# NVIDIA/tensorrt-laboratory

Measured on NVIDIA H100. Metric: ResNet-50 fp16 b=8 inferences/sec, higher is better.
Workload: dtype f16

## Files before the change

### tensorrt_laboratory_b200/csrc/engine.cu

```cuda
#include <cuda.h>
#include <cuda_runtime.h>
#include <stdarg.h>
#include <stdio.h>
#include <stdlib.h>
#include <string.h>

#include <algorithm>
#include <map>
#include <memory>
#include <mutex>
#include <string>
#include <vector>

#include "../../include/b200infer.h"
#include "kernels.h"
#include "plan_format.h"

#include "b2_internal.h"

namespace b2i {
thread_local std::string g_err;
int fail(int code, const char* fmt, ...) {
    char buf[1024];
    va_list ap;
// ... 42 lines not shown
        if (cudaGetDriverEntryPoint("cuTensorMapEncodeIm2col", &fn, cudaEnableDefault, &q) != cudaSuccess || !fn) {
            g_driver_status = 2;
            return;
        }
        g_encode_im2col = reinterpret_cast<EncodeIm2colFn>(fn);
        cudaDriverGetVersion(&g_driver_version);
    });
    return g_driver_status;
}

size_t align_up(size_t v, size_t a) { return (v + a - 1) / a * a; }
constexpr size_t kSplitWorkspaceBytes = 12u << 20;
constexpr int kMaxSplitTiles = 4096;

int env_int(const char* name, int dflt) {
    const char* v = getenv(name);
    return v ? atoi(v) : dflt;
}

struct Tensor {
    std::string name;
    uint32_t kind, h, w, c, c_phys;
    int binding;
    float scale = 0.f;
    size_t item_bytes = 0;
    size_t offset = 0;
    int def = -1, last_use = -1;
};

struct Op {
    b2plan::OpRec r;
    std::string name;
    int side_join = -1;
    int kh() const { return int(r.k); }
    int kw() const { return int(r.kw ? r.kw : r.k); }
    int sh() const { return int(r.stride); }
    int sw() const { return int(r.kw ? r.stride_w : r.stride); }
    int ph() const { return int(r.pad_); }
    int pw_lo() const { return int(r.kw ? r.pad_w_lo : r.pad_); }
    int pw_hi() const { return int(r.kw ? r.pad_w_hi : r.pad_); }
    double algo_k() const { return r.ceil_mode ? double(r.ceil_mode) : double(r.cin) * r.taps; }
};

struct Binding {
    std::string name;
    bool is_input;
    int dtype;
    int tensor;
    int nd;
    int32_t dims[8];
    size_t item_bytes;
};

enum LKind { L_INPUT_CAST, L_CONV_TC, L_CONV_SIMT, L_MAXPOOL, L_AVGPOOL, L_FC, L_SOFTMAX, L_OUTPUT_CAST, L_NET, L_TAIL, L_QUANTIZE, L_CONV_I8, L_AVGPOOL_I8, L_OUTPUT_CAST_I8 };

struct NetRun {
    b2k::NetArgs args{};
    int ctas = 0;
    int first_op = 0, last_op = 0;
    void* d_blob = nullptr;
    ~NetRun() {
        if (d_blob) cudaFree(d_blob);
    }
};

struct Launch {
    LKind kind;
    std::string name;
    double flops = 0, bytes = 0;
    b2k::ConvLaunch conv;
    b2k::SimtConvArgs simt;
    const void* in = nullptr;
    void* out = nullptr;
    const void* w = nullptr;
    const float* bias = nullptr;
    int in_binding = -1, out_binding = -1;
    bool src_half = false;
    int max_blocks = 0;
    int side_join = -1;
    std::shared_ptr<NetRun> net;
    b2k::TailArgs tail{};
    b2k::I8ConvLaunch i8{};
    float qscale = 0.f;
    int C_in_phys = 0;
    bool net_member = false;
    int N = 0, C = 0, H = 0, W = 0, C_phys = 0, Ho = 0, Wo = 0, k = 0, stride = 0, pad = 0, K = 0, Cout = 0;
};

struct Segment {
    int begin = 0, end = 0;
    bool graphable = false;
    cudaGraphExec_t exec = nullptr;
};
struct BindPatch {
    int launch = -1;
    cudaGraphNode_t node = nullptr;
    cudaKernelNodeParams np{};
    std::vector<void*> params;
    int n_params = 0;
    int in_index = -1, out_index = -1;
    void* in_value = nullptr;
    void* out_value = nullptr;
    b2k::TailArgs tail{};
    bool is_tail = false;
};
struct Plan {
    int batch = 0;
    bool has_net = false;
    std::vector<Launch> launches;
    std::vector<Segment> segments;
    bool graph_failed = false;
    cudaGraph_t graph = nullptr;
    cudaGraphExec_t exec = nullptr;
    std::vector<BindPatch> patches;
    ~Plan() {
        for (Segment& sg : segments)
            if (sg.exec) cudaGraphExecDestroy(sg.exec);
        if (exec) cudaGraphExecDestroy(exec);
        if (graph) cudaGraphDestroy(graph);
    }
};

}

struct ConvConfig {
    int bn, stages, splits;
    double est_us;
    int sps = 1;
    int ws = 0;
    int cn = 1;
    int halo = 0;
};
static bool stage_depth_useful(int bn, int kb, int st, int kpc) {
    const int stgs[4] = {1, 2, 4, 8};
    int cover = 0, deepest = 0;
// ... 14 lines not shown
    void* user = nullptr;
};

struct b2_engine {
    b2_runtime* rt = nullptr;
    b2_alloc_fn alloc = nullptr;
    b2_free_fn free_ = nullptr;
    void* alloc_user = nullptr;
    std::string name;
    int precision = 0, max_batch = 0;
    std::vector<Tensor> tensors;
    std::vector<Op> ops;
    std::vector<Binding> bindings;
    uint8_t* d_payload = nullptr;
    size_t payload_bytes = 0;
    size_t arena_bytes = 0;
    size_t act_bytes = 0;
    int device = -1;
    bool inspect_only = false;
    double flops_per_item = 0;
    std::mutex tune_mutex;
    std::mutex tune_run_mutex;
    std::map<std::pair<int, int>, ConvConfig> tuned;
    bool tune_cache_loaded = false;
    std::map<int, float> requant_r;
    bool tactics_from_plan = false;
    bool tuned_at_load = false;
    bool half() const { return precision != B2_PREC_FP32; }
    bool int8() const { return precision == B2_PREC_INT8; }
};

struct b2_context {
    b2_engine* e = nullptr;
    uint8_t* scratch = nullptr;
    struct ScratchState {
        std::map<int, std::unique_ptr<Plan>> plans;
    };
    std::map<uint8_t*, ScratchState> states;
    ScratchState* cur = nullptr;
    int* d_counters = nullptr;
    int use_graph = 1;
    int force_simt = 0;
    int force_im2col = 0;
    int force_bn = 0;
    int force_stages = 0;
    int force_splits = 0;
    int force_sps = 0;
    int force_halo = 0;
    int force_cn = 0;
    int force_ws = 0;
    int pdl_trigger = 1;
    int no_pack = 0;
    int no_fold = 0;
    int autotune = 4;
    int fork = 0;
    int net = 0;
    int net_ctas = 0;
    int net_bn = 0;
    int net_stages = 0;
    int i8_bn = 0;
    int i8_stages = 0;
    int fuse_tail = 1;
    int input_ctas = 0;
    int* d_tail_ctrl = nullptr;
    cudaStream_t side = nullptr;
    cudaEvent_t fork_ev = nullptr, join_ev = nullptr;
};

namespace {

std::string fixed_str(const char* p, size_t n) {
    size_t len = 0;
    while (len < n && p[len]) ++len;
    return std::string(p, len);
}

int parse_blob(const void* blob, size_t nbytes, b2_engine* e, const uint8_t** payload) {
    using namespace b2plan;
    if (!blob || nbytes < sizeof(Header)) return fail(B2_EINVAL, "plan: blob too small (%zu bytes)", nbytes);
    const uint8_t* base = static_cast<const uint8_t*>(blob);
    Header h;
    memcpy(&h, base, sizeof h);
    if (memcmp(h.magic, kMagic, 8) != 0) return fail(B2_EINVAL, "plan: bad magic (not a B2ENGINE blob)");
    if (h.version != kVersion) return fail(B2_EINVAL, "plan: version %u, this library reads %u", h.version, kVersion);
    if (h.precision > 2) return fail(B2_EINVAL, "plan: unknown precision %u", h.precision);
    if (h.max_batch == 0 || h.max_batch > 4096) return fail(B2_EINVAL, "plan: bad max_batch %u", h.max_batch);
    const size_t tbl = sizeof(Header) + size_t(h.n_tensors) * sizeof(TensorRec) + size_t(h.n_ops) * sizeof(OpRec) +
                       size_t(h.n_bindings) * sizeof(BindingRec);
    if (tbl > nbytes || h.payload_offset < tbl || h.payload_offset > nbytes || h.payload_bytes > nbytes - h.payload_offset)
        return fail(B2_EINVAL, "plan: truncated (tables %zu, payload %llu+%llu, blob %zu)", tbl,
                    (unsigned long long)h.payload_offset, (unsigned long long)h.payload_bytes, nbytes);
    e->name = fixed_str(h.name, 64);
    e->precision = h.precision;
    e->max_batch = h.max_batch;
    e->payload_bytes = h.payload_bytes;
    const size_t elt = h.precision == B2_PREC_FP32 ? 4 : 2;
    const uint8_t* p = base + sizeof(Header);
    for (uint32_t i = 0; i < h.n_tensors; ++i, p += sizeof(TensorRec)) {
        TensorRec r;
        memcpy(&r, p, sizeof r);
        Tensor t;
        t.name = fixed_str(r.name, 64);
        t.kind = r.kind;
        t.h = r.h, t.w = r.w, t.c = r.c, t.c_phys = r.c_phys;
        t.binding = r.binding;
        t.scale = h.precision == B2_PREC_INT8 ? r.scale : 0.f;
// ... 228 lines not shown
    if (g_driver_version <= 13010 && img_bytes * uint64_t(N) < 131072)
        reinterpret_cast<uint64_t*>(map)[1] &= ~(1ull << 21);
    return B2_OK;
}

static int g_sms = 132;

ConvConfig pick_conv_config(int M, int cout_phys, int kblocks, int kb, bool residual, const b2_context* c, bool honor_forced) {
    const int m_tiles = (M + 127) / 128;
    ConvConfig best{0, 0, 1, 1e30};
    const int bns[4] = {256, 128, 64, 32};
    const int stgs[4] = {1, 2, 4, 8};
    for (int bn : bns) {
        if (cout_phys % bn) continue;
        if (honor_forced && c->force_bn && bn != c->force_bn) continue;
        const int tiles = m_tiles * (cout_phys / bn);
        for (int splits = 1; splits <= 8; ++splits) {
            if (c->force_splits ? splits != c->force_splits : splits != 1) continue;
            if (splits > 1 && (kb != 64 || kblocks / splits < 4 || tiles * splits > 160 || tiles > kMaxSplitTiles ||
                               size_t(tiles) * splits * 128 * bn * 4 > kSplitWorkspaceBytes))
                continue;
            const int kpc = (kblocks + splits - 1) / splits;
            if (splits > 1 && (splits - 1) * kpc >= kblocks) continue;
            for (int st : stgs) {
                if (!b2k::conv_config_exists(bn, kb, st)) continue;
                if (b2k::conv_smem_bytes(bn, st, residual) > 227 * 1024) continue;
                if (honor_forced && c->force_stages && st != c->force_stages) continue;
                if (!(honor_forced && c->force_stages) && !stage_depth_useful(bn, kb, st, kpc)) continue;
                const double smem = b2k::conv_smem_bytes(bn, st, residual);
                int per_sm = int(227.0 * 1024 / smem);
                per_sm = std::min(per_sm, bn <= 64 ? 2 : 1);
                per_sm = std::max(1, std::min(per_sm, 8));
                const int ctas = tiles * splits;
                const int waves = (ctas + g_sms * per_sm - 1) / (g_sms * per_sm);
                const int sharing = std::max(1, std::min(per_sm, (ctas + g_sms - 1) / g_sms));
                const double stage_bytes = 16384.0 + bn * 128.0;
                const double t_kb = std::max(stage_bytes / (70000.0 / sharing), 1.0 / st);
                double t_epi = 0.6 + bn / 64.0 * 0.4 + (residual ? 0.4 : 0.0);
                if (splits > 1) t_epi += 1.0 + 0.3 * splits;
                const double t_cta = 2.0 + kpc * t_kb + t_epi;
                double total = waves * t_cta;
                const double traffic = double(ctas) * kpc * stage_bytes;
                total = std::max(total, traffic / 5.0e6 + 2.0);
                if (total < best.est_us) best = ConvConfig{bn, st, splits, total};
            }
        }
    }
    return best;
}

bool conv_is_row_folded(const b2_context* c, const Op& op) {
    const b2plan::OpRec& r = op.r;
    return !c->no_fold && r.cin_phys == 8 && op.kw() * 8 * 2 == 64 && op.sw() == 1 && op.pw_lo() == 0 && op.pw_hi() == 0;
}
int conv_kb(const b2_context* c, const Op& op) {
    if (op.r.cin_phys % 64 == 0) return 64;
    return conv_is_row_folded(c, op) ? 32 : 8;
}
int conv_num_kblocks(const b2_context* c, const Op& op) {
    const b2plan::OpRec& r = op.r;
    if (r.cin_phys % 64 == 0) return int(r.taps) * (int(r.cin_phys) / 64);
    if (conv_is_row_folded(c, op)) return (op.kh() + 1) / 2;
    return (int(r.taps_phys) + 7) / 8;
}

int conv_halo_rows(const b2_context* c, const Op& op) {
    const b2plan::OpRec& r = op.r;
    const Tensor& ti = c->e->tensors[r.in];
    const Tensor& to = c->e->tensors[r.out];
    if (r.cin_phys % 64 || r.cout_phys % 64 || op.kh() != 3 || op.kw() != 3 || op.sh() != 1 || op.sw() != 1 || op.ph() != 1 ||
        op.pw_lo() != 1 || op.pw_hi() != 1 || r.res >= 0 || !(r.relu & 2) || c->no_pack || ti.h != to.h || ti.w != to.w)
        return 0;
    const int wp = int(to.w) + 2;
    if (wp > 128) return 0;
    return std::min(128 / wp, int(to.h));
}

int make_conv_launch(b2_context* c, const Op& op, int batch, const ConvConfig& cfg, b2k::ConvLaunch* out) {
    b2_engine* e = c->e;
    const b2plan::OpRec& r = op.r;
    const Tensor& ti = e->tensors[r.in];
    const Tensor& to = e->tensors[r.out];
    auto tptr = [&](int idx) -> uint8_t* { return c->scratch + e->tensors[idx].offset; };
    const uint8_t* w = e->d_payload + r.w_off;
    const int M = batch * int(to.h) * int(to.w);
    const bool kb64 = r.cin_phys % 64 == 0;
    const bool fold = conv_is_row_folded(c, op);
    b2k::ConvLaunch& cl = *out;
    memset(&cl, 0, sizeof cl);
    cl.kb = conv_kb(c, op);
    cl.grid_m = (M + 127) / 128;
    const int nkb = conv_num_kblocks(c, op);
    cl.bn = cfg.bn;
    cl.stages = cfg.stages;
    cl.sps = cfg.sps > 0 ? cfg.sps : 1;
    cl.grid_n = int(r.cout_phys) / cl.bn;
    cl.ws_ctas = cfg.ws;
    cl.cn = (cfg.cn > 1 && cfg.ws == 0 && cl.kb == 64 && cl.grid_n % cfg.cn == 0 &&
             b2k::conv_cluster_config_exists(cl.bn, cl.stages, cl.sps, cfg.cn)) ? cfg.cn : 1;
    cl.args.cn = cl.cn;
    cl.args.tiles_m = cl.grid_m;
    cl.args.tiles_n = cl.grid_n;
    b2k::ConvArgs& a = cl.args;
    a.splits = cfg.splits;
    a.kb_per_split = (nkb + cfg.splits - 1) / cfg.splits;
    a.workspace = reinterpret_cast<float*>(c->scratch + e->act_bytes);
// ... 646 lines not shown
                L.bytes = double(batch) * t.h * t.w * (t.c * 4.0 + t.c_phys * elt);
                break;
            }
            case b2plan::OP_QUANTIZE: {
                const Tensor& ti = e->tensors[r.in];
                const Tensor& to = e->tensors[r.out];
                L.kind = L_QUANTIZE;
                L.in = tptr(r.in), L.out = tptr(r.out);
                L.C = ti.c, L.H = ti.h, L.W = ti.w, L.C_in_phys = ti.c_phys, L.C_phys = to.c_phys;
                L.qscale = float(1.0 / double(to.scale));
                L.bytes = double(batch) * (ti.item_bytes + to.item_bytes);
                break;
            }
            case b2plan::OP_OUTPUT_CAST: {
                const Tensor& t = e->tensors[r.in];
                L.kind = t.scale > 0.f ? L_OUTPUT_CAST_I8 : L_OUTPUT_CAST;
                L.qscale = t.scale;
                L.in = tptr(r.in);
                L.out_binding = r.binding;
                L.C = t.c, L.H = t.h, L.W = t.w, L.C_phys = t.c_phys;
                L.bytes = double(batch) * t.h * t.w * (t.c * 4.0 + t.c_phys * elt);
                break;
            }
            case b2plan::OP_CONV: {
                const Tensor& ti = e->tensors[r.in];
                const Tensor& to = e->tensors[r.out];
                const uint8_t* w = e->d_payload + r.w_off;
                const float* bias = reinterpret_cast<const float*>(e->d_payload + r.b_off);
                const int M = batch * int(to.h) * int(to.w);
                L.flops = 2.0 * M * r.cout * op.algo_k();
                L.bytes = double(batch) * (ti.item_bytes + to.item_bytes * (r.res >= 0 ? 2 : 1)) + double(r.w_bytes);
                const bool kb64 = r.cin_phys % 64 == 0;
                const bool kb8 = r.cin_phys == 8;
                const bool tc_ok = half && !c->force_simt && (kb64 || kb8) && r.cout_phys % 32 == 0 &&
                                   (kb64 || r.taps_phys % 2 == 0);
                if (r.relu & 4) {
                    L.kind = L_CONV_I8;
                    const int m_tiles = (batch * int(e->tensors[r.out].h * e->tensors[r.out].w) + 127) / 128;
                    int bn = 128, st = m_tiles * (int(r.cout_phys) / 128) >= 2 * g_sms ? 1 : 2;
                    if (c->autotune) {
                        std::lock_guard<std::mutex> lock(e->tune_mutex);
                        tune_cache_load(e);
                        const int op_index = int(&op - &e->ops[0]);
                        auto it = e->tuned.find({op_index, batch});
                        if (it == e->tuned.end()) it = e->tuned.find({op_index, e->max_batch});
                        if (it != e->tuned.end()) bn = it->second.bn, st = it->second.stages;
                    }
                    if (c->i8_bn > 0) bn = c->i8_bn;
                    if (c->i8_stages > 0) st = c->i8_stages;
                    if (int(r.cout_phys) % bn) bn = 128;
                    if (!b2k::conv_i8_config_exists(bn, st)) bn = 128, st = 2;
                    int rc = make_i8_conv_launch(c, op, batch, bn, st, &L.i8);
                    if (rc) return rc;
                } else if (tc_ok) {
                    L.kind = L_CONV_TC;
                    const int kbsz = conv_kb(c, op);
                    const int nkb = conv_num_kblocks(c, op);
                    ConvConfig cfg = pick_conv_config(M, int(r.cout_phys), nkb, kbsz, r.res >= 0, c, true);
                    if (cfg.bn == 0)
                        cfg = pick_conv_config(M, int(r.cout_phys), nkb, kbsz, r.res >= 0, c, false);
                    if (cfg.bn == 0) return fail(B2_EINVAL, "conv %s: no kernel configuration", op.name.c_str());
                    if (c->force_sps == 2 && b2k::conv_config_exists(cfg.bn, kbsz, cfg.stages, 2) &&
                        b2k::conv_smem_bytes(cfg.bn, cfg.stages, r.res >= 0, 2) <= 227 * 1024)
                        cfg.sps = 2;
                    if (c->force_ws > 0 && kbsz == 64 && (r.relu & 2) && cfg.splits == 1 &&
                        b2k::conv_ws_config_exists(cfg.bn, cfg.stages, cfg.sps) &&
                        b2k::conv_ws_smem(cfg.bn, cfg.stages, cfg.sps, r.res >= 0) <= 227 * 1024)
                        cfg.ws = std::min(((M + 127) / 128) * (int(r.cout_phys) / cfg.bn), c->force_ws > 1 ? c->force_ws : g_sms);
                    if (c->force_halo > 0 && conv_halo_rows(c, op) && b2k::conv_halo_config_exists(cfg.bn) && cfg.splits == 1 &&
                        int(r.cin_phys) / 64 <= 8 && b2k::conv_halo_smem(cfg.bn, int(to.w), conv_halo_rows(c, op), int(r.cin_phys) / 64) <= 227 * 1024)
                        cfg.halo = 1, cfg.ws = 0, cfg.cn = 1;
                    if (c->force_cn > 1 && kbsz == 64 && cfg.ws == 0 && !cfg.halo && (int(r.cout_phys) / cfg.bn) % c->force_cn == 0) cfg.cn = c->force_cn;
                    const bool forced = c->force_bn || c->force_stages || c->force_splits || c->force_sps;
                    const int op_index = int(&op - &e->ops[0]);
                    const bool net_ok = c->net && !forced && kbsz == 64 && (r.relu & 2) && !c->no_pack && r.cout_phys % 64 == 0 &&
                                        c->force_ws <= 0 && c->force_cn <= 0 && c->force_halo <= 0 && !c->force_im2col;
                    if (net_ok) {
                        int bn = (r.cout_phys % 128 == 0) ? 128 : 64;
                        if (c->net_bn == 64) bn = 64;
                        cfg = ConvConfig{bn, 4, 1, 0.0, 1, 0, 1};
                        cfg.halo = 0;
                        L.net_member = true;
                    } else if (!forced && c->autotune) {
                        std::lock_guard<std::mutex> lock(e->tune_mutex);
                        tune_cache_load(e);
                        auto it = e->tuned.find({op_index, batch});
                        if (it == e->tuned.end()) it = e->tuned.find({op_index, e->max_batch});
                        if (it != e->tuned.end() && tactic_applies(c, op, batch, it->second)) cfg = it->second;
                    }
                    if (op.side_join >= 0 && cfg.splits > 1) cfg.splits = 1;
                    int rc = make_conv_launch(c, op, batch, cfg, &L.conv);
                    if (rc) return rc;
                } else {
                    L.kind = L_CONV_SIMT;
                    b2k::SimtConvArgs& a = L.simt;
                    memset(&a, 0, sizeof a);
                    a.in = tptr(r.in), a.w = w, a.bias = bias;
                    a.residual = r.res >= 0 ? tptr(r.res) : nullptr;
                    a.out = tptr(r.out);
                    a.N = batch, a.H = int(ti.h), a.W = int(ti.w), a.Cin = int(r.cin), a.Cin_phys = int(r.cin_phys);
                    a.Ho = int(to.h), a.Wo = int(to.w), a.Cout = int(r.cout), a.Cout_phys = int(r.cout_phys);
                    a.kh = op.kh(), a.kw = op.kw(), a.taps_phys = int(r.taps_phys);
                    a.stride_h = op.sh(), a.stride_w = op.sw(), a.pad_h = op.ph(), a.pad_w = op.pw_lo();
                    a.relu = int(r.relu & 1);
                    a.w_packed = int((r.relu >> 1) & 1);
                }
// ... 38 lines not shown
            }
            case b2plan::OP_SOFTMAX: {
                const Tensor& ti = e->tensors[r.in];
                const Tensor& to = e->tensors[r.out];
                L.kind = L_SOFTMAX;
                L.in = tptr(r.in);
                L.in_binding = ti.binding;
                L.out = tptr(r.out);
                L.out_binding = to.binding;
                L.C = int(ti.c);
                L.bytes = double(batch) * ti.c * 8.0;
                break;
            }
            default:
                return fail(B2_EINVAL, "op %s: unknown type", op.name.c_str());
        }
        plan->launches.push_back(std::move(L));
    }
    int rc = fuse_net_runs(c, plan.get(), batch);
    if (rc) return rc;
    fuse_tail(c, plan.get(), batch);
    {
        const std::vector<Launch>& ls = plan->launches;
        size_t i = 0;
        while (i < ls.size()) {
            const bool dep = ls[i].in_binding >= 0 || ls[i].out_binding >= 0;
            size_t j = i + 1;
            if (!dep)
                while (j < ls.size() && ls[j].in_binding < 0 && ls[j].out_binding < 0) ++j;
            Segment sg;
            sg.begin = int(i), sg.end = int(j);
            sg.graphable = !dep && (j - i) >= 3 && !plan->has_net;
            plan->segments.push_back(sg);
            i = j;
        }
    }
    *out = plan.get();
    c->cur->plans[batch] = std::move(plan);
    return B2_OK;
}

int run_launch(const b2_engine* e, const Launch& L, void* const* bindings, cudaStream_t s) {
    const bool half = e->half();
    const void* in = L.in_binding >= 0 ? bindings[L.in_binding] : L.in;
    void* out = L.out_binding >= 0 ? bindings[L.out_binding] : L.out;
    switch (L.kind) {
        case L_INPUT_CAST:
            if (L.k == 2) return b2k::launch_input_cast_s2d(in, L.src_half, out, L.N, L.C, L.H, L.W, L.pad, L.stride, L.max_blocks, s);
            return b2k::launch_input_cast(in, L.src_half, out, L.N, L.C, L.H, L.W, L.C_phys, half, L.max_blocks, s);
        case L_OUTPUT_CAST:
            return b2k::launch_output_cast(in, static_cast<float*>(out), L.N, L.C, L.H, L.W, L.C_phys, half, s);
        case L_CONV_TC:
            return b2k::launch_conv_f16_tcgen05(L.conv, s);
        case L_CONV_SIMT:
            return b2k::launch_conv_simt(L.simt, half, s);
        case L_MAXPOOL:
            return b2k::launch_maxpool(in, out, L.N, L.H, L.W, L.C_phys, L.Ho, L.Wo, L.k, L.stride, L.pad, half, s);
        case L_AVGPOOL:
            return b2k::launch_avgpool(in, out, L.N, L.H * L.W, L.C_phys, half, s);
        case L_FC:
            return b2k::launch_fc(in, L.w, L.bias, static_cast<float*>(out), L.N, L.K, L.Cout, half, s);
        case L_SOFTMAX:
            return b2k::launch_softmax(static_cast<const float*>(in), static_cast<float*>(out), L.N, L.C, s);
        case L_NET:
            return b2k::launch_net_f16_tcgen05(L.net->args, L.net->ctas, s);
        case L_QUANTIZE:
            return b2k::launch_quantize_h_to_i8(in, out, static_cast<long long>(L.N) * L.H * L.W, L.C, L.C_in_phys, L.C_phys, L.qscale, s);
        case L_CONV_I8:
            return b2k::launch_conv_i8_tcgen05(L.i8, s);
        case L_AVGPOOL_I8:
            return b2k::launch_avgpool_i8(in, out, L.N, L.H * L.W, L.C, L.C_in_phys, L.C_phys, L.qscale, s);
        case L_OUTPUT_CAST_I8:
            return b2k::launch_output_cast_i8(in, static_cast<float*>(out), L.N, L.C, L.H, L.W, L.C_phys, L.qscale, s);
        case L_TAIL: {
            b2k::TailArgs t = L.tail;
            t.out = static_cast<float*>(out);
            return b2k::launch_tail_f16(t, s);
        }
    }
    return int(cudaErrorInvalidValue);
}

int run_range(b2_context* c, const Plan& plan, size_t first, size_t last, void* const* bindings, cudaStream_t s);
int run_all(b2_context* c, const Plan& plan, void* const* bindings, cudaStream_t s) {
    return run_range(c, plan, 0, plan.launches.size(), bindings, s);
}
int run_range(b2_context* c, const Plan& plan, size_t first, size_t last, void* const* bindings, cudaStream_t s) {
    const b2_engine* e = c->e;
    bool fork = c->fork != 0;
    if (fork && !c->side) {
        if (cudaStreamCreateWithFlags(&c->side, cudaStreamNonBlocking) != cudaSuccess ||
            cudaEventCreateWithFlags(&c->fork_ev, cudaEventDisableTiming) != cudaSuccess ||
            cudaEventCreateWithFlags(&c->join_ev, cudaEventDisableTiming) != cudaSuccess) {
            cudaGetLastError();
            fork = false;
        }
    }
    int pending_join = -1;
    for (size_t i = first; i < last; ++i) {
        const Launch& L = plan.launches[i];
        if (pending_join == int(i)) {
            B2_CUDA(cudaStreamWaitEvent(s, c->join_ev, 0));
            pending_join = -1;
        }
        int rc;
        if (fork && pending_join < 0 && L.side_join > int(i) && L.side_join < int(last)) {
// ... 323 lines not shown
    c->cur = c->scratch ? &c->states[c->scratch] : nullptr;
}

void b2_context_destroy(b2_context* c) {
    if (!c) return;
    drop_cached(c);
    if (c->d_counters) cudaFree(c->d_counters);
    if (c->side) cudaStreamDestroy(c->side);
    if (c->fork_ev) cudaEventDestroy(c->fork_ev);
    if (c->join_ev) cudaEventDestroy(c->join_ev);
    delete c;
}

int b2_context_set_device_memory(b2_context* c, void* scratch) {
    if (!c || !scratch) return fail(B2_EINVAL, "null context or scratch");
    if (reinterpret_cast<uintptr_t>(scratch) % 256 != 0) return fail(B2_EINVAL, "scratch must be 256-byte aligned (cudaMalloc alignment)");
    if (c->states.size() >= 32 && c->states.find(static_cast<uint8_t*>(scratch)) == c->states.end()) drop_cached(c);
    c->scratch = static_cast<uint8_t*>(scratch);
    c->cur = &c->states[c->scratch];
    return B2_OK;
}

int b2_context_set_option(b2_context* c, const char* key, int value) {
    if (!c || !key) return fail(B2_EINVAL, "null context or key");
    const std::string k(key);
    if (k == "graph") {
        c->use_graph = value;
        return B2_OK;
    }
    if (k == "pdl") {
        b2k::set_pdl(value != 0);
        value = 0;
    } else if (k == "simt") c->force_simt = value;
    else if (k == "im2col") c->force_im2col = value;
    else if (k == "bn") c->force_bn = value;
    else if (k == "stages") c->force_stages = value;
    else if (k == "splits") c->force_splits = value;
    else if (k == "sps") c->force_sps = value;
    else if (k == "ws") c->force_ws = value;
    else if (k == "cn") c->force_cn = value;
    else if (k == "halo") c->force_halo = value;
    else if (k == "fork") c->fork = value;
    else if (k == "net") c->net = value;
    else if (k == "net_ctas") c->net_ctas = value;
    else if (k == "net_bn") c->net_bn = value;
    else if (k == "net_stages") c->net_stages = value;
    else if (k == "fuse_tail") c->fuse_tail = value;
    else if (k == "i8_bn") c->i8_bn = value;
    else if (k == "i8_stages") c->i8_stages = value;
    else if (k == "input_ctas") c->input_ctas = value;
    else if (k == "pdl_trigger") c->pdl_trigger = value;
    else if (k == "autotune") c->autotune = value;
    else if (k == "no_fold") c->no_fold = value;
    else return fail(B2_EINVAL, "unknown option '%s'", key);
    drop_cached(c);
    return B2_OK;
}

int b2_context_nb_launches(b2_context* c, int batch) {
    if (!c) return -1;
    Plan* plan = nullptr;
    if (build_plan(c, batch, &plan)) return -1;
    return int(plan->launches.size());
}

int b2_engine_tune(b2_engine* e, int streams, int all_batches) {
    if (!e) return fail(B2_EINVAL, "null engine");
    if (e->inspect_only) return fail(B2_ESTATE, "engine was loaded with b2_engine_inspect (no device resources)");
    if (!e->half() || e->tactics_from_plan) return B2_OK;
    std::lock_guard<std::mutex> run_lock(e->tune_run_mutex);
    b2_context* c = nullptr;
    int rc = b2_context_create(e, &c);
    if (rc) return rc;
    c->autotune = streams > 0 ? streams : c->autotune;
    void* scratch = nullptr;
    if (c->autotune <= 0) {
        b2_context_destroy(c);
        return B2_OK;
    }
    if (cudaMalloc(&scratch, std::max<size_t>(e->arena_bytes, 1024)) != cudaSuccess) {
        cudaGetLastError();
        b2_context_destroy(c);
        return fail(B2_ENOMEM, "cudaMalloc(%zu) for the tuning arena failed", e->arena_bytes);
    }
    rc = b2_context_set_device_memory(c, scratch);
    if (!rc && load_driver_entry_points() != 0) rc = fail(B2_ECUDA, "cuTensorMapEncode* driver entry points unavailable");
    {
        std::lock_guard<std::mutex> lock(e->tune_mutex);
        tune_cache_load(e);
    }
    if (!rc) rc = tune_engine_batch(c, e->max_batch);
    for (int b = 1; !rc && all_batches && b < e->max_batch; ++b) rc = tune_engine_batch(c, b);
    cudaDeviceSynchronize();
    b2_context_destroy(c);
    cudaFree(scratch);
    if (!rc) e->tuned_at_load = true;
    return rc;
}

namespace {
struct RefineCtx {
    b2_context* c = nullptr;
    void* scratch = nullptr;
    std::vector<void*> bind;
    cudaStream_t s = nullptr;
};
// ... 264 lines not shown
    Plan* plan = nullptr;
    if (!c || build_plan(c, batch, &plan)) return fail(B2_EINVAL, "no plan");
    if (i < 0 || i >= int(plan->launches.size()) || plan->launches[i].kind != L_CONV_TC) return fail(B2_EINVAL, "not a tcgen05 conv launch");
    b2k::ConvLaunch cl = plan->launches[i].conv;
    const int ctas = cl.ws_ctas > 0 ? cl.ws_ctas : cl.grid_m * cl.grid_n * cl.args.splits;
    if (n_ctas) *n_ctas = ctas;
    if (ctas > cap_ctas) return fail(B2_EINVAL, "stamp buffer too small (%d CTAs)", ctas);
    long long* d = nullptr;
    B2_CUDA(cudaMalloc(&d, size_t(ctas) * 16 * sizeof(long long)));
    cudaMemset(d, 0, size_t(ctas) * 16 * sizeof(long long));
    cl.args.dbg = d;
    cl.args.dbg_mode = dbg_mode;
    cudaStream_t s = static_cast<cudaStream_t>(stream_);
    int rc = 0;
    for (int r = 0; r < reps && !rc; ++r) rc = b2k::launch_conv_f16_tcgen05(cl, s);
    cudaError_t se = cudaStreamSynchronize(s);
    if (!rc && se == cudaSuccess) cudaMemcpy(stamps, d, size_t(ctas) * 16 * sizeof(long long), cudaMemcpyDeviceToHost);
    cudaFree(d);
    if (rc || se != cudaSuccess) return fail(B2_ECUDA, "debug launch failed: %s", cudaGetErrorString(rc ? cudaError_t(rc) : se));
    return B2_OK;
}

int b2_context_debug_net_timing(b2_context* c, int batch, void* const* bindings, b2_stream_t stream_, long long* out, int cap_ctas,
                                int* n_ctas) {
    Plan* plan = nullptr;
    if (!c || build_plan(c, batch, &plan)) return fail(B2_EINVAL, "no plan");
    NetRun* run = nullptr;
    for (Launch& L : plan->launches)
        if (L.kind == L_NET) run = L.net.get();
    if (!run) return fail(B2_EINVAL, "the plan has no persistent network kernel");
    if (n_ctas) *n_ctas = run->ctas;
    if (run->ctas > cap_ctas) return fail(B2_EINVAL, "counter buffer too small (%d CTAs)", run->ctas);
    long long* d = nullptr;
    const size_t bytes = size_t(run->ctas) * 64 * sizeof(long long);
    B2_CUDA(cudaMalloc(&d, bytes));
    cudaMemset(d, 0, bytes);
    cudaStream_t s = static_cast<cudaStream_t>(stream_);
    run->args.dbg = d;
    int rc = run_all(c, *plan, bindings, s);
    cudaError_t se = cudaStreamSynchronize(s);
    run->args.dbg = nullptr;
    if (!rc && se == cudaSuccess) cudaMemcpy(out, d, bytes, cudaMemcpyDeviceToHost);
    cudaFree(d);
    if (rc) return rc;
    if (se != cudaSuccess) return fail(B2_ECUDA, "debug launch failed: %s", cudaGetErrorString(se));
    return B2_OK;
}

const char* b2_context_launch_name(b2_context* c, int batch, int i) {
    static thread_local std::string s;
    const Launch* L = get_launch(c, batch, i);
    if (!L) return nullptr;
    static const char* kinds[] = {"input_cast", "conv_tcgen05", "conv_simt", "maxpool", "avgpool", "fc", "softmax", "output_cast", "net_tcgen05", "tail_pool_fc_softmax",
                                  "quantize", "conv_i8_tcgen05", "avgpool_i8", "output_cast_i8"};
    s = std::string(kinds[L->kind]) + ":" + L->name;
    if (L->kind == L_CONV_TC)
        s += " bn=" + std::to_string(L->conv.bn) + " kb=" + std::to_string(L->conv.kb) +
             " st=" + std::to_string(L->conv.stages) + "x" + std::to_string(L->conv.sps) +
             (L->conv.ws_ctas ? " ws=" + std::to_string(L->conv.ws_ctas) : std::string()) +
             (L->conv.cn > 1 ? " cn=" + std::to_string(L->conv.cn) : std::string()) + (L->conv.halo ? " halo" : "") +
             (L->conv.args.a_mode == b2k::A_TILED ? " tiled" : " im2col") +
             " grid=" + std::to_string(L->conv.grid_n) + "x" + std::to_string(L->conv.grid_m) + "x" +
             std::to_string(L->conv.args.splits) + " kblk=" + std::to_string(L->conv.args.num_kblocks);
    if (L->kind == L_CONV_I8)
        s += " bn=" + std::to_string(L->i8.bn) + " st=" + std::to_string(L->i8.stages) + (L->i8.args.a_mode == b2k::A_TILED ? " tiled" : " im2col") + " grid=" +
             std::to_string(L->i8.grid_n) + "x" + std::to_string(L->i8.grid_m) + " kblk=" + std::to_string(L->i8.args.num_kblocks);
    if (L->kind == L_NET)
        s += " layers=" + std::to_string(L->net->args.n_layers) + " tiles=" + std::to_string(L->net->args.total_tiles) +
             " ctas=" + std::to_string(L->net->ctas) + " stages=" + std::to_string(L->net->args.stages);
    if (L->side_join >= 0) s += " side";
    return s.c_str();
}
double b2_context_launch_flops(b2_context* c, int batch, int i) {
    const Launch* L = get_launch(c, batch, i);
    return L ? L->flops : 0.0;
}
double b2_context_launch_bytes(b2_context* c, int batch, int i) {
    const Launch* L = get_launch(c, batch, i);
    return L ? L->bytes : 0.0;
}

}
```

### tensorrt_laboratory_b200/csrc/kernels.cu

```cuda
#include "kernels.h"

#include <stdio.h>
#include <stdlib.h>
#include <string.h>

#include "ptx_sm90.cuh"
#include "wgmma_sm90.cuh"

namespace b2k {

template <int BN, int STAGES, int SPS = 1>
struct ConvCfg {
    static constexpr int A_SUBBLK = 128 * 64 * 2;
    static constexpr int B_SUBBLK = BN * 64 * 2;
    static constexpr int A_STAGE = SPS * A_SUBBLK;
    static constexpr int B_STAGE = SPS * B_SUBBLK;
    static constexpr int PIPE_BYTES = STAGES * (A_STAGE + B_STAGE);
    static constexpr int TILE_BYTES = 128 * BN * 2;
    static_assert(TILE_BYTES <= PIPE_BYTES, "the output staging tile reuses the pipeline buffers");
};

__host__ __device__ constexpr int conv_smem_layout_bytes(int bn, int stages, bool residual, int sps = 1) {
    return stages * sps * (128 * 64 * 2 + bn * 64 * 2) + (residual ? 128 * bn * 2 : 0) + 256 + bn * 4 + 1024;
}
// ... 846 lines not shown
        if constexpr (KB == 64) {
            if ((e = static_cast<int>(cudaFuncSetAttribute(conv_f16_tcgen05<BN, KB, STAGES, SPS, 1, false, 1>,
                                                           cudaFuncAttributeMaxDynamicSharedMemorySize, bytes)))) return e;
            if ((e = static_cast<int>(cudaFuncSetAttribute(conv_f16_tcgen05<BN, KB, STAGES, SPS, 1, false, 2>,
                                                           cudaFuncAttributeMaxDynamicSharedMemorySize, bytes)))) return e;
        }
    }
    return static_cast<int>(cudaFuncSetAttribute(conv_f16_tcgen05<BN, KB, STAGES, SPS, CN>, cudaFuncAttributeMaxDynamicSharedMemorySize, bytes));
}

int conv_smem_bytes(int bn, int stages, bool residual, int sps) { return conv_smem_layout_bytes(bn, stages, residual, sps); }

#define B2_FOR_EACH_CONV(X) \
    X(32, 64, 1, 1) X(32, 64, 2, 1) X(32, 64, 4, 1) X(32, 64, 8, 1) \
    X(64, 64, 1, 1) X(64, 64, 2, 1) X(64, 64, 4, 1) X(64, 64, 8, 1) \
    X(128, 64, 1, 1) X(128, 64, 2, 1) X(128, 64, 4, 1) X(256, 64, 2, 1) X(256, 64, 4, 1) \
    X(32, 64, 2, 2) X(32, 64, 4, 2) X(64, 64, 2, 2) X(64, 64, 4, 2) X(128, 64, 2, 2) X(256, 64, 2, 2) \
    X(32, 8, 2, 1) X(32, 8, 4, 1) X(64, 8, 2, 1) X(64, 8, 4, 1) X(64, 8, 8, 1) X(128, 8, 4, 1) \
    X(32, 32, 2, 1) X(32, 32, 4, 1) X(64, 32, 1, 1) X(64, 32, 2, 1) X(64, 32, 4, 1) X(128, 32, 2, 1) X(128, 32, 4, 1)

int conv_halo_smem(int bn, int w, int r, int cblocks) { return halo_smem_bytes(bn, w, r, cblocks); }
bool conv_halo_config_exists(int bn) { return bn == 64 || bn == 128 || bn == 256; }
static int init_conv_halo_kernels() {
    int e;
    if ((e = static_cast<int>(cudaFuncSetAttribute(conv3x3_halo_tcgen05<64>, cudaFuncAttributeMaxDynamicSharedMemorySize, 227 * 1024)))) return e;
    if ((e = static_cast<int>(cudaFuncSetAttribute(conv3x3_halo_tcgen05<128>, cudaFuncAttributeMaxDynamicSharedMemorySize, 227 * 1024)))) return e;
    if ((e = static_cast<int>(cudaFuncSetAttribute(conv3x3_halo_tcgen05<256>, cudaFuncAttributeMaxDynamicSharedMemorySize, 227 * 1024)))) return e;
    return 0;
}
static int launch_conv_halo(const ConvLaunch& L, cudaStream_t stream) {
    const int R = L.args.halo_rows;
    const size_t smem = size_t(halo_smem_bytes(L.bn, L.args.Wo, R, L.args.cblocks));
    if (smem > 227 * 1024 || R < 1 || R * (L.args.Wo + 2) > 128 || L.args.cblocks > kHaloMaxCBlocks) return static_cast<int>(cudaErrorInvalidValue);
    dim3 grid(L.grid_n, L.grid_m, 1);
    switch (L.bn) {
        case 64: return launch_kernel(conv3x3_halo_tcgen05<64>, grid, dim3(kConvThreads), smem, stream, true, L.mapA, L.mapOut, L.args);
        case 128: return launch_kernel(conv3x3_halo_tcgen05<128>, grid, dim3(kConvThreads), smem, stream, true, L.mapA, L.mapOut, L.args);
        case 256: return launch_kernel(conv3x3_halo_tcgen05<256>, grid, dim3(kConvThreads), smem, stream, true, L.mapA, L.mapOut, L.args);
    }
    return static_cast<int>(cudaErrorInvalidValue);
}

#define B2_FOR_EACH_CONV_CLUSTER(X) \
    X(32, 4, 1, 2) X(32, 4, 1, 4) X(64, 1, 1, 2) X(64, 2, 1, 2) X(64, 2, 1, 4) X(64, 2, 2, 2) X(64, 4, 2, 2) X(64, 4, 2, 4) \
    X(128, 2, 1, 2) X(128, 2, 1, 4) X(128, 2, 2, 2)

int init_conv_ws_kernels();
int launch_conv_f16_tcgen05_ws(const ConvLaunch& L, cudaStream_t stream);

int init_conv_kernels() {
    int e = init_conv_ws_kernels();
    if (e) return e;
    if ((e = init_conv_halo_kernels())) return e;
#define B2_INIT(BN_, KB_, ST_, SPS_) \
    if ((e = init_one<BN_, KB_, ST_, SPS_>())) return e;
    B2_FOR_EACH_CONV(B2_INIT)
#undef B2_INIT
#define B2_INIT_CL(BN_, ST_, SPS_, CN_) \
    if ((e = init_one<BN_, 64, ST_, SPS_, CN_>())) return e;
    B2_FOR_EACH_CONV_CLUSTER(B2_INIT_CL)
#undef B2_INIT_CL
    return 0;
}

int launch_conv_f16_tcgen05(const ConvLaunch& L, cudaStream_t stream) {
    if (L.halo) return launch_conv_halo(L, stream);
    if (L.ws_ctas > 0) return launch_conv_f16_tcgen05_ws(L, stream);
    if (L.cn > 1) {
#define B2_CASE_CL(BN_, ST_, SPS_, CN_) \
    if (L.bn == BN_ && L.kb == 64 && L.stages == ST_ && L.sps == SPS_ && L.cn == CN_) return launch_one<BN_, 64, ST_, SPS_, CN_>(L, stream);
        B2_FOR_EACH_CONV_CLUSTER(B2_CASE_CL)
#undef B2_CASE_CL
        return static_cast<int>(cudaErrorInvalidValue);
    }
#define B2_CASE(BN_, KB_, ST_, SPS_) \
    if (L.bn == BN_ && L.kb == KB_ && L.stages == ST_ && L.sps == SPS_) return launch_one<BN_, KB_, ST_, SPS_>(L, stream);
    B2_FOR_EACH_CONV(B2_CASE)
#undef B2_CASE
    return static_cast<int>(cudaErrorInvalidValue);
}

#define B2_FOR_EACH_CONV_WS(X) \
    X(32, 4, 1) X(64, 2, 1) X(64, 4, 1) X(64, 2, 2) X(64, 4, 2) X(128, 2, 1) X(128, 4, 1) X(128, 2, 2)

template <int BN, int STAGES, int SPS>
static int launch_one_ws(const ConvLaunch& L, cudaStream_t stream) {
    const size_t smem = size_t(conv_ws_smem_bytes(BN, STAGES, SPS, L.args.residual != nullptr));
    return launch_kernel(conv_f16_tcgen05_ws<BN, STAGES, SPS>, dim3(L.ws_ctas), dim3(kConvThreads), smem, stream, true, L.mapA, L.mapOut,
                         L.mapRes, L.args);
}

int init_conv_ws_kernels() {
    int e = 0;
#define B2_INIT_WS(BN_, ST_, SPS_)                                                                                        \
    {                                                                                                                     \
        const int want = conv_ws_smem_bytes(BN_, ST_, SPS_, true);                                                        \
        e = static_cast<int>(cudaFuncSetAttribute(conv_f16_tcgen05_ws<BN_, ST_, SPS_>,                                    \
                                                  cudaFuncAttributeMaxDynamicSharedMemorySize,                            \
                                                  want > 227 * 1024 ? conv_ws_smem_bytes(BN_, ST_, SPS_, false) : want)); \
        if (e) return e;                                                                                                  \
    }
    B2_FOR_EACH_CONV_WS(B2_INIT_WS)
#undef B2_INIT_WS
    return 0;
}

// ... 819 lines not shown
```

### tensorrt_laboratory_b200/csrc/kernels.h

```cpp
#pragma once
#include <cuda.h>
#include <cuda_fp16.h>
#include <cuda_runtime.h>
#include <stdint.h>

namespace b2k {

enum { A_TILED = 0, A_IM2COL = 1 };

struct ConvArgs {
    const float* bias;
    const __half* residual;
    __half* out;
    int M;
    int Cout;
    int num_kblocks;
    int cblocks;
    int taps;
    int taps_phys;
    int kw;
    int HoWo, Wo;
    int stride_h, stride_w;
    int pad_h, pad_w;
    int relu;
    int a_mode;
    int splits;
    int kb_per_split;
    float* workspace;
    int* tile_counters;
    int pdl_trigger;
    const uint8_t* wpacked;
    int halo_rows;
    int cn;
    int tiles_m, tiles_n;
    int dbg_mode;
    long long* dbg;
};

struct ConvLaunch {
    CUtensorMap mapA;
    CUtensorMap mapB;
    CUtensorMap mapOut;
    CUtensorMap mapRes;
    ConvArgs args;
    int bn;
    int kb;
    int stages;
    int sps;
    int grid_m, grid_n;
    int cn;
    int halo;
    int ws_ctas;
};

int launch_conv_f16_tcgen05(const ConvLaunch& L, cudaStream_t stream);
int init_conv_kernels();
bool conv_config_exists(int bn, int kb, int stages, int sps = 1);
int conv_smem_bytes(int bn, int stages, bool residual, int sps = 1);
bool conv_cluster_config_exists(int bn, int stages, int sps, int cn);
bool conv_halo_config_exists(int bn);
int conv_halo_smem(int bn, int w, int r, int cblocks);
bool conv_ws_config_exists(int bn, int stages, int sps);
int conv_ws_smem(int bn, int stages, int sps, bool residual);
void set_pdl(bool on);
bool get_pdl();

constexpr int kNetMaxLayers = 160;

struct NetLayerInfo {
    const uint8_t* wpacked;
    const float* bias;
    __half* out;
    const __half* residual;
    int M, Cout, num_kblocks, cblocks;
    int kw, HoWo, Wo, stride_h;
    int stride_w, pad_h, pad_w, relu;
    int a_mode, bn, tiles_m, tiles_n;
    int tile_begin, total_tiles;
    int in_flag_off;
    int in_need;
    int res_flag_off, res_need;
    int out_flag_off;
    int dep_off;
    int war_upto;
    int pad_[3];
};
static_assert(sizeof(NetLayerInfo) % 16 == 0, "NetLayerInfo is copied to shared memory in 16-byte words");
struct alignas(64) NetLayer {
    CUtensorMap mapA;
    NetLayerInfo info;
};
struct NetArgs {
    const NetLayer* layers;
    const short2* deps;
    int* mt_done;
    int* layer_done;
    int* ctrl;
    int n_layers, total_tiles, n_flags;
    int stages;
    long long* dbg;
};
int init_net_kernel();
int net_smem_bytes(int n_layers, int stages);
int launch_net_f16_tcgen05(const NetArgs& a, int ctas, cudaStream_t stream);

struct I8ConvArgs {
    const uint8_t* wpacked;
    const float* m;
    const float* b;
    float r;
    int has_res, relu;
    int M, Cout, num_kblocks, cblocks;
    int kw, HoWo, Wo, stride_h, stride_w, pad_h, pad_w, a_mode;
    int last_cb_mmas, cout_real;
};
struct I8ConvLaunch {
// ... 56 lines not shown
```

Baseline: 30050.

## Add dedicated banded wgmma kernel for the row-folded 7x7 stem convolution

Adds a specialised stem convolution kernel that loads a band of input rows into shared memory once with a bulk copy, keeps the 7x7 weights resident, and computes several output rows per CTA with wgmma, reusing the overlapping input rows. It writes outputs through a swizzled shared staging buffer and supports PDL. It replaces the generic implicit-GEMM tcgen05 path for the stem when the shape matches (cout 64, kh 7, row-folded, no residual, width up to 128), aiming to cut redundant input loads and per-k-block pipeline overhead. The risk is lower parallelism, only Ho/4 x N CTAs, and a large shared-memory footprint per CTA.

```diff
diff --git a/tensorrt_laboratory_b200/csrc/engine.cu b/tensorrt_laboratory_b200/csrc/engine.cu
--- a/tensorrt_laboratory_b200/csrc/engine.cu
+++ b/tensorrt_laboratory_b200/csrc/engine.cu
@@ -118,7 +118,8 @@
     size_t item_bytes;
 };
 
-enum LKind { L_INPUT_CAST, L_CONV_TC, L_CONV_SIMT, L_MAXPOOL, L_AVGPOOL, L_FC, L_SOFTMAX, L_OUTPUT_CAST, L_NET, L_TAIL, L_QUANTIZE, L_CONV_I8, L_AVGPOOL_I8, L_OUTPUT_CAST_I8 };
+enum LKind { L_INPUT_CAST, L_CONV_TC, L_CONV_SIMT, L_MAXPOOL, L_AVGPOOL, L_FC, L_SOFTMAX, L_OUTPUT_CAST, L_NET, L_TAIL, L_QUANTIZE, L_CONV_I8, L_AVGPOOL_I8, L_OUTPUT_CAST_I8,
+             L_CONV_STEM };
 
 struct NetRun {
     b2k::NetArgs args{};
@@ -147,6 +148,7 @@
     std::shared_ptr<NetRun> net;
     b2k::TailArgs tail{};
     b2k::I8ConvLaunch i8{};
+    b2k::StemConvArgs stem{};
     float qscale = 0.f;
     int C_in_phys = 0;
     bool net_member = false;
@@ -267,6 +269,7 @@
     int pdl_trigger = 1;
     int no_pack = 0;
     int no_fold = 0;
+    int no_stem_band = 0;
     int autotune = 4;
     int fork = 0;
     int net = 0;
@@ -601,6 +604,11 @@
 bool conv_is_row_folded(const b2_context* c, const Op& op) {
     const b2plan::OpRec& r = op.r;
     return !c->no_fold && r.cin_phys == 8 && op.kw() * 8 * 2 == 64 && op.sw() == 1 && op.pw_lo() == 0 && op.pw_hi() == 0;
+}
+bool conv_is_stem_band(const b2_context* c, const Op& op) {
+    const b2plan::OpRec& r = op.r;
+    return !c->no_stem_band && conv_is_row_folded(c, op) && r.cout_phys == 64 && op.kh() == 7 && r.taps_phys == r.taps &&
+           r.res < 0 && !(r.relu & 2) && c->e->tensors[r.out].w <= 128;
 }
 int conv_kb(const b2_context* c, const Op& op) {
     if (op.r.cin_phys % 64 == 0) return 64;
@@ -1353,6 +1361,18 @@
                     if (!b2k::conv_i8_config_exists(bn, st)) bn = 128, st = 2;
                     int rc = make_i8_conv_launch(c, op, batch, bn, st, &L.i8);
                     if (rc) return rc;
+                } else if (tc_ok && conv_is_stem_band(c, op)) {
+                    L.kind = L_CONV_STEM;
+                    b2k::StemConvArgs& a = L.stem;
+                    a.in = tptr(r.in), a.w = reinterpret_cast<const __half*>(w), a.bias = bias;
+                    a.out = reinterpret_cast<uint4*>(tptr(r.out));
+                    a.Ho = int(to.h), a.Wo = int(to.w), a.stride_h = op.sh(), a.pad_h = op.ph(), a.relu = int(r.relu & 1);
+                    a.rows = 4;
+                    a.band_rows = (a.rows - 1) * a.stride_h + op.kh();
+                    a.in_row_bytes = int(ti.w) * 16;
+                    a.N = batch, a.H = int(ti.h);
+                    if (b2k::conv_stem_band_smem(a.band_rows, a.in_row_bytes, a.Wo) > 227 * 1024)
+                        return fail(B2_EINVAL, "conv %s: input rows too wide for the stem kernel", op.name.c_str());
                 } else if (tc_ok) {
                     L.kind = L_CONV_TC;
                     const int kbsz = conv_kb(c, op);
@@ -1497,6 +1517,8 @@
             return b2k::launch_output_cast(in, static_cast<float*>(out), L.N, L.C, L.H, L.W, L.C_phys, half, s);
         case L_CONV_TC:
             return b2k::launch_conv_f16_tcgen05(L.conv, s);
+        case L_CONV_STEM:
+            return b2k::launch_conv_stem_band(L.stem, s);
         case L_CONV_SIMT:
             return b2k::launch_conv_simt(L.simt, half, s);
         case L_MAXPOOL:
@@ -1926,6 +1948,7 @@
     else if (k == "pdl_trigger") c->pdl_trigger = value;
     else if (k == "autotune") c->autotune = value;
     else if (k == "no_fold") c->no_fold = value;
+    else if (k == "no_stem_band") c->no_stem_band = value;
     else return fail(B2_EINVAL, "unknown option '%s'", key);
     drop_cached(c);
     return B2_OK;
@@ -2296,7 +2319,7 @@
     const Launch* L = get_launch(c, batch, i);
     if (!L) return nullptr;
     static const char* kinds[] = {"input_cast", "conv_tcgen05", "conv_simt", "maxpool", "avgpool", "fc", "softmax", "output_cast", "net_tcgen05", "tail_pool_fc_softmax",
-                                  "quantize", "conv_i8_tcgen05", "avgpool_i8", "output_cast_i8"};
+                                  "quantize", "conv_i8_tcgen05", "avgpool_i8", "output_cast_i8", "conv_tcgen05"};
     s = std::string(kinds[L->kind]) + ":" + L->name;
     if (L->kind == L_CONV_TC)
         s += " bn=" + std::to_string(L->conv.bn) + " kb=" + std::to_string(L->conv.kb) +
@@ -2312,6 +2335,9 @@
     if (L->kind == L_NET)
         s += " layers=" + std::to_string(L->net->args.n_layers) + " tiles=" + std::to_string(L->net->args.total_tiles) +
              " ctas=" + std::to_string(L->net->ctas) + " stages=" + std::to_string(L->net->args.stages);
+    if (L->kind == L_CONV_STEM)
+        s += " stem band rows=" + std::to_string(L->stem.rows) + " grid=" + std::to_string((L->stem.Ho + L->stem.rows - 1) / L->stem.rows) + "x" +
+             std::to_string(L->stem.N);
     if (L->side_join >= 0) s += " side";
     return s.c_str();
 }
diff --git a/tensorrt_laboratory_b200/csrc/kernels.cu b/tensorrt_laboratory_b200/csrc/kernels.cu
--- a/tensorrt_laboratory_b200/csrc/kernels.cu
+++ b/tensorrt_laboratory_b200/csrc/kernels.cu
@@ -922,6 +922,7 @@
     int e = init_conv_ws_kernels();
     if (e) return e;
     if ((e = init_conv_halo_kernels())) return e;
+    if ((e = init_conv_stem_band())) return e;
 #define B2_INIT(BN_, KB_, ST_, SPS_) \
     if ((e = init_one<BN_, KB_, ST_, SPS_>())) return e;
     B2_FOR_EACH_CONV(B2_INIT)
diff --git a/tensorrt_laboratory_b200/csrc/kernels.h b/tensorrt_laboratory_b200/csrc/kernels.h
--- a/tensorrt_laboratory_b200/csrc/kernels.h
+++ b/tensorrt_laboratory_b200/csrc/kernels.h
@@ -62,6 +62,22 @@
 int conv_halo_smem(int bn, int w, int r, int cblocks);
 bool conv_ws_config_exists(int bn, int stages, int sps);
 int conv_ws_smem(int bn, int stages, int sps, bool residual);
+struct StemConvArgs {
+    const uint8_t* in;
+    const __half* w;
+    const float* bias;
+    uint4* out;
+    int Ho, Wo;
+    int stride_h, pad_h;
+    int relu;
+    int rows;
+    int band_rows;
+    int in_row_bytes;
+    int N, H;
+};
+int init_conv_stem_band();
+int conv_stem_band_smem(int band_rows, int in_row_bytes, int wo);
+int launch_conv_stem_band(const StemConvArgs& a, cudaStream_t stream);
 void set_pdl(bool on);
 bool get_pdl();
 
diff --git a/tensorrt_laboratory_b200/csrc/stem_conv.cu b/tensorrt_laboratory_b200/csrc/stem_conv.cu
--- /dev/null
+++ b/tensorrt_laboratory_b200/csrc/stem_conv.cu
@@ -0,0 +1,132 @@
+#include "kernels.h"
+
+#include "ptx_sm90.cuh"
+#include "wgmma_sm90.cuh"
+
+namespace b2k {
+
+constexpr int kStemThreads = 256;
+constexpr int kStemKH = 7;
+constexpr int kStemWBytes = kStemKH * 4 * 1024;
+constexpr int kStemOverread = 2048;
+
+__host__ __device__ constexpr int stem_in_region(int band_rows, int in_row_bytes) {
+    return (band_rows * in_row_bytes + kStemOverread + 1023) / 1024 * 1024;
+}
+__host__ __device__ constexpr int stem_smem_bytes(int band_rows, int in_row_bytes, int wo) {
+    return stem_in_region(band_rows, in_row_bytes) + kStemWBytes + 2 * wo * 128 + 256 + 16 + 1024;
+}
+
+__global__ void __launch_bounds__(kStemThreads, 2)
+conv_stem_band_f16(const StemConvArgs p) {
+    extern __shared__ uint8_t smem_raw[];
+    uint8_t* smem = smem_raw + ((1024u - (smem_u32(smem_raw) & 1023u)) & 1023u);
+    uint8_t* sIn = smem;
+    uint8_t* sB = smem + stem_in_region(p.band_rows, p.in_row_bytes);
+    uint8_t* sOut = sB + kStemWBytes;
+    const int slot_bytes = p.Wo * 128;
+    float* s_bias = reinterpret_cast<float*>(sOut + 2 * slot_bytes);
+    uint64_t* in_bar = reinterpret_cast<uint64_t*>(s_bias + 64);
+
+    const int img = blockIdx.y;
+    const int o_lo = blockIdx.x * p.rows;
+    const int o_hi = min(p.Ho, o_lo + p.rows);
+    const int r_lo = o_lo * p.stride_h - p.pad_h;
+    const int v_lo = max(r_lo, 0), v_hi = min(r_lo + p.band_rows, p.H);
+
+    if (threadIdx.x == 0) {
+        mbar_init(in_bar, 1);
+        fence_barrier_init();
+    }
+    {
+        const int n16 = p.in_row_bytes / 16;
+        const int top = (v_lo - r_lo) * n16, bottom = (r_lo + p.band_rows - v_hi) * n16;
+        uint4* dst = reinterpret_cast<uint4*>(sIn);
+        uint4* dst_b = reinterpret_cast<uint4*>(sIn + (v_hi - r_lo) * p.in_row_bytes);
+        for (int i = threadIdx.x; i < top; i += kStemThreads) dst[i] = make_uint4(0u, 0u, 0u, 0u);
+        for (int i = threadIdx.x; i < bottom; i += kStemThreads) dst_b[i] = make_uint4(0u, 0u, 0u, 0u);
+    }
+    const uint4* wsrc = reinterpret_cast<const uint4*>(p.w);
+    for (int i = threadIdx.x; i < 64 * kStemKH * 4; i += kStemThreads) {
+        const int n = i / (kStemKH * 4), kc = i - n * (kStemKH * 4);
+        *reinterpret_cast<uint4*>(sB + kc * 1024 + n * 16) = __ldg(wsrc + i);
+    }
+    if (threadIdx.x < 64) s_bias[threadIdx.x] = __ldg(p.bias + threadIdx.x);
+    fence_proxy_async();
+    __syncthreads();
+
+    pdl_wait();
+    if (threadIdx.x == 0) {
+        const uint32_t bytes = static_cast<uint32_t>((v_hi - v_lo) * p.in_row_bytes);
+        mbar_expect_tx(in_bar, bytes);
+        bulk_load_1d(in_bar, sIn + (v_lo - r_lo) * p.in_row_bytes, p.in + (static_cast<size_t>(img) * p.H + v_lo) * p.in_row_bytes, bytes);
+    }
+    mbar_wait(in_bar, 0);
+    pdl_launch_dependents();
+
+    const int wg = threadIdx.x >> 7;
+    const int warp = (threadIdx.x >> 5) & 3, lane = threadIdx.x & 31;
+    const uint32_t a_base = smem_u32(sIn) + static_cast<uint32_t>(wg * 64 * 16);
+    const uint32_t b_base = smem_u32(sB);
+    const int q_frag = 64 * wg + 16 * warp + (lane >> 2);
+    const int col_frag = 2 * (lane & 3);
+    float acc[32];
+#pragma unroll 1
+    for (int orow = o_lo; orow < o_hi; ++orow) {
+        const uint32_t a_row = a_base + static_cast<uint32_t>((orow - o_lo) * p.stride_h * p.in_row_bytes);
+        wgmma_group<2 * kStemKH>([&](int t) {
+            const int r = t >> 1, j = t & 1;
+            const uint64_t ad = make_wgmma_desc(a_row + static_cast<uint32_t>(r * p.in_row_bytes + j * 32), 16, 128, WG_NOSWZ);
+            const uint64_t bd = make_wgmma_desc(b_base + static_cast<uint32_t>((4 * r + 2 * j) * 1024), 1024, 128, WG_NOSWZ);
+            wgmma_f16<64>(acc, ad, bd, t > 0 ? 1u : 0u);
+        });
+        wgmma_wait<0>();
+
+        uint8_t* slot = sOut + (orow & 1) * slot_bytes;
+#pragma unroll
+        for (int h = 0; h < 2; ++h) {
+            const int q = q_frag + 8 * h;
+            if (q >= p.Wo) continue;
+#pragma unroll
+            for (int j = 0; j < 8; ++j) {
+                const int col = 8 * j + col_frag;
+                float v0 = acc[4 * j + 2 * h] + s_bias[col], v1 = acc[4 * j + 2 * h + 1] + s_bias[col + 1];
+                if (p.relu) {
+                    v0 = fmaxf(v0, 0.0f);
+                    v1 = fmaxf(v1, 0.0f);
+                }
+                *reinterpret_cast<__half2*>(slot + q * 128 + ((j ^ (q & 7)) << 4) + col_frag * 2) = __floats2half2_rn(v0, v1);
+            }
+        }
+        __syncthreads();
+        uint4* dst = p.out + (static_cast<size_t>(img) * p.Ho + orow) * p.Wo * 8;
+        for (int it = threadIdx.x; it < p.Wo * 8; it += kStemThreads) {
+            const int q = it >> 3, c = it & 7;
+            dst[it] = *reinterpret_cast<const uint4*>(slot + q * 128 + ((c ^ (q & 7)) << 4));
+        }
+    }
+}
+
+int conv_stem_band_smem(int band_rows, int in_row_bytes, int wo) { return stem_smem_bytes(band_rows, in_row_bytes, wo); }
+
+int init_conv_stem_band() {
+    return static_cast<int>(cudaFuncSetAttribute(conv_stem_band_f16, cudaFuncAttributeMaxDynamicSharedMemorySize, 227 * 1024));
+}
+
+int launch_conv_stem_band(const StemConvArgs& a, cudaStream_t stream) {
+    const size_t smem = size_t(stem_smem_bytes(a.band_rows, a.in_row_bytes, a.Wo));
+    if (smem > 227 * 1024 || a.rows < 1 || a.Wo > 128 || a.in_row_bytes % 16) return static_cast<int>(cudaErrorInvalidValue);
+    cudaLaunchConfig_t cfg = {};
+    cfg.gridDim = dim3(static_cast<unsigned>((a.Ho + a.rows - 1) / a.rows), static_cast<unsigned>(a.N));
+    cfg.blockDim = dim3(kStemThreads);
+    cfg.dynamicSmemBytes = smem;
+    cfg.stream = stream;
+    cudaLaunchAttribute attr[1];
+    attr[0].id = cudaLaunchAttributeProgrammaticStreamSerialization;
+    attr[0].val.programmaticStreamSerializationAllowed = 1;
+    cfg.attrs = attr;
+    cfg.numAttrs = get_pdl() ? 1 : 0;
+    return static_cast<int>(cudaLaunchKernelEx(&cfg, conv_stem_band_f16, a));
+}
+
+}
```

New measurement: 30830 (median of 6 runs). 1.03x the previous value.
